# boyuanf/tensorflow_train_distributed

Hardware: AMD Instinct MI355X
Metric: images/sec (whole node) ResNet-50 bf16 MirroredStrategy at 1/2/4/8 MI355X (higher is better)
Workload: dtype bf16; 1 GPU; model=ResNet-50 v1.5, global_batch=1024, per_gpu_batch=1024, image_size=224, parallelism=dp1, optimizer=momentum-SGD 0.9, wd 5e-5, fp32 master, precision=bf16, hipgraph=True

## Files before the change

### tensorflow_train_distributed_amd/csrc/kernels/conv3_halo.hip

```cpp
#include "stream_epi.h"

namespace ttdk {
namespace {
namespace c3 {

constexpr int THR = 512;
constexpr int NW = THR / 64;

struct Pro {
  const bf16_t* x;
  const bf16_t* x2;
  const uint8_t* mask;
  const float* s;
  const float* b;
  bf16_t* side;
  uint8_t* side_mask;
};

__device__ __forceinline__ void load8f(const float* p, float (&d)[8]) {
  const f32x4_t a = *reinterpret_cast<const f32x4_t*>(p), c = *reinterpret_cast<const f32x4_t*>(p + 4);
#pragma unroll
  for (int j = 0; j < 4; ++j) {
    d[j] = a[j];
    d[4 + j] = c[j];
  }
}

template <int CP>
__device__ __forceinline__ int slot_chunk(int q) { return (q >> 3) % CP; }
template <int CP>
__device__ __forceinline__ int slot_pix(int q) { return (q & 7) + 8 * (q / (8 * CP)); }

template <int SCHED>
__device__ __forceinline__ int fresh(int tid) {
  if constexpr (SCHED != 0) {
    asm volatile("" : "+v"(tid));
    __builtin_assume(tid >= 0 && tid < THR);
  }
  return tid;
}

template <int SCHED>
__device__ __forceinline__ void frag_fence() {
  if constexpr (SCHED != 0) __builtin_amdgcn_sched_barrier(0);
}

template <int C, int BN, int TH, int W, int PRO, bool FLIP, int WM, int SCHED, int FEED>
__global__ __launch_bounds__(THR, 1) void conv3_kernel(Pro pa, const bf16_t* __restrict__ w, EpiParams E, int H,
                                                      int N, int tiles, int nslices) {
  constexpr int BM = TH * W;
  constexpr int HR = TH + 2, HC = W + 2;
  constexpr int CP = C / 8;
  constexpr int KT = 9 * C;
  constexpr int WN = NW / WM;
  constexpr int WR = BM / WM, WC = BN / WN;
  constexpr int TM = WR / 16, TN = WC / 16;
  constexpr int NPIX = HR * HC;
  constexpr int NCH = ((NPIX + 7) / 8) * 8 * CP;
  constexpr int NA = (NCH + THR - 1) / THR;
  constexpr int SB = BN * KT * 2;
  constexpr int REG = ((NPIX * 16 + 255) / 256) * 256;
  constexpr int SH = CP * REG;
  constexpr int PITCH = BN * 2 + 16;
  constexpr int SE = BM * PITCH + NW * 3 * BN * 4;
  constexpr int SAE = SH > SE ? SH : SE;
  static_assert(C % 64 == 0 && BN % 32 == 0 && WR % 16 == 0 && WC % 16 == 0, "tile shape");
  static_assert(THR % (8 * CP) == 0, "fixed channel chunk per thread");
  static_assert(SB + SAE <= 160 * 1024, "LDS budget");
  __shared__ __attribute__((aligned(16))) char smem[SB + SAE];
  char* const sB = smem;
  char* const sA = smem + SB;

  const int b = blockIdx.x;
  const int G = gridDim.x / nslices;
  const int xcd = b & 7, rq = b >> 3;
  const int slice = rq % nslices;
  const int per_xcd = G / 8;
  const int g = xcd * per_xcd + rq / nslices;
  const int n0 = slice * BN;
  const int tid = threadIdx.x, lane = tid & 63, wave = tid >> 6;
  const int wm = wave / WN, wn = wave % WN;
  const int tiles_per_img = H / TH;

  for (int q = tid; q < BN * (KT / 8); q += THR) {
    const int row = q / (KT / 8), kk = q % (KT / 8);
    const int tap = kk / CP, cc = kk % CP;
    const int n = n0 + row;
    const int src_tap = FLIP ? 8 - tap : tap;
    const uint4 v = n < N ? ldg16(w + (static_cast<long long>(n) * 9 + src_tap) * C + cc * 8) : make_uint4(0, 0, 0, 0);
    *reinterpret_cast<uint4*>(sB + (kk >> 3) * (BN * 128) + kmaj_off(row, kk & 7)) = v;
  }

  const int ac = slot_chunk<CP>(tid);
  const bool write_side = slice == 0 && pa.side != nullptr;

  const char* abase[TM];
#pragma unroll
  for (int a = 0; a < TM; ++a) {
    const int i = wm * WR + a * 16 + (lane & 15);
    abase[a] = sA + (lane >> 4) * REG + ((i / W) * HC + (i % W)) * 16;
  }

  uint4 ra[NA], rx[PRO == 2 ? NA : 1];
  uint32_t rm[(NA + 3) / 4];
  auto load_tile = [&](int t) {
    const int img = t / tiles_per_img, h0 = (t % tiles_per_img) * TH;
    const int ft = fresh<SCHED>(tid);
#pragma unroll
    for (int i = 0; i < (NA + 3) / 4; ++i) rm[i] = 0;
#pragma unroll
    for (int i = 0; i < NA; ++i) {
      const int pix = slot_pix<CP>(ft + THR * i);
      const int hr = pix / HC, hc = pix % HC;
      const int h = h0 - 1 + hr, x = hc - 1;
      const bool ok = pix < NPIX && h >= 0 && h < H && x >= 0 && x < W;
      const long long off = ((static_cast<long long>(img) * H + h) * W + x) * C + ac * 8;
      ra[i] = ok ? ldg16(pa.x + off) : make_uint4(0, 0, 0, 0);
      if constexpr (PRO == 2) {
        rx[i] = ok ? ldg16(pa.x2 + off) : make_uint4(0, 0, 0, 0);
        rm[i >> 2] |= static_cast<uint32_t>((ok && pa.mask) ? pa.mask[off >> 3] : 0xffu) << (8 * (i & 3));
      }
    }
  };
  auto stage_tile = [&](int t) {
    const int img = t / tiles_per_img, h0 = (t % tiles_per_img) * TH;
    float k0[8], k1[8], k2[8];
    if constexpr (PRO == 1) {
      load8f(pa.s + ac * 8, k0);
      load8f(pa.b + ac * 8, k1);
    } else if constexpr (PRO == 2) {
      load8f(pa.s + ac * 8, k0);
      load8f(pa.s + C + ac * 8, k1);
      load8f(pa.s + 2 * C + ac * 8, k2);
    }
    const int ft = fresh<SCHED>(tid);
#pragma unroll
    for (int i = 0; i < NA; ++i) {
      const int pix = slot_pix<CP>(ft + THR * i);
      if (ft + THR * i >= NCH) break;
      const int hr = pix / HC, hc = pix % HC;
      const int h = h0 - 1 + hr, x = hc - 1;
      const bool ok = h >= 0 && h < H && x >= 0 && x < W;
      const bool interior = ok && hr >= 1 && hr <= TH;
      const long long off = ((static_cast<long long>(img) * H + h) * W + x) * C + ac * 8;
      uint4 v = ra[i];
      if constexpr (PRO == 1) {
        float f[8];
        unpack8(ra[i], f);
#pragma unroll
        for (int j = 0; j < 8; ++j) f[j] = relu(f[j] * k0[j] + k1[j]);
        v = ok ? pack8(f) : make_uint4(0, 0, 0, 0);
        if (write_side && interior) {
          *reinterpret_cast<uint4*>(pa.side + off) = v;
          if (pa.side_mask) {
            const uint32_t wv[4] = {v.x, v.y, v.z, v.w};
            uint32_t mb = 0;
#pragma unroll
            for (int j = 0; j < 8; ++j) {
              const uint32_t hb = (wv[j >> 1] >> (16 * (j & 1))) & 0xffffu;
              mb |= ((hb & 0x7fffu) != 0 && !(hb & 0x8000u) ? 1u : 0u) << j;
            }
            pa.side_mask[off >> 3] = static_cast<uint8_t>(mb);
          }
        }
      } else if constexpr (PRO == 2) {
        float gq[8], yf[8];
        unpack8(ra[i], gq);
        const uint32_t mb = rm[i >> 2] >> (8 * (i & 3));
#pragma unroll
        for (int j = 0; j < 8; ++j) gq[j] = (mb >> j) & 1u ? gq[j] : 0.f;
        unpack8(rx[i], yf);
#pragma unroll
        for (int j = 0; j < 8; ++j) gq[j] = k0[j] * gq[j] + k1[j] * yf[j] + k2[j];
        v = ok ? pack8(gq) : make_uint4(0, 0, 0, 0);
        if (write_side && interior) *reinterpret_cast<uint4*>(pa.side + off) = v;
      }
      *reinterpret_cast<uint4*>(sA + ac * REG + pix * 16) = v;
    }
  };

  constexpr int ECPR = BN / 8;
  constexpr int RPP = THR / ECPR;
  constexpr int NR = (BM + RPP - 1) / RPP;
  constexpr int FA = NR >= 6 ? 3 : 2, FTAP = 6;
  static_assert(FEED == 0 || (FLIP && SCHED != 0), "feeding epilogue: data gradients under SCHED 1");
  const int M = tiles * BM;

  int t = g;
  if (t < tiles) load_tile(t);
  for (; t < tiles; t += G) {
    stage_tile(t);
    __syncthreads();
    if (t + G < tiles) load_tile(t + G);
    const int m0 = t * BM;
    sepi::FeedBatch<FA> fa;
    sepi::FeedBatch<NR - FA> fb;
    f32x4_t acc[TM][TN];
#pragma unroll
    for (int a = 0; a < TM; ++a)
#pragma unroll
      for (int c = 0; c < TN; ++c) acc[a][c] = f32x4_t{0.f, 0.f, 0.f, 0.f};
#pragma unroll
    for (int tap = 0; tap < 9; ++tap) {
      const int tq = (tap / 3) * HC + (tap % 3);
#pragma unroll
      for (int kc = 0; kc < C / 32; ++kc) {
        if constexpr (FEED != 0) {
          if (tap == FTAP && kc == 0) {
            const int ft = fresh<SCHED>(tid);
            sepi::feed_batch_load<BM, RPP, FA>(fa, E, 0, ft / ECPR, m0, M, n0 + (ft % ECPR) * 8);
          }
        }
        const int kglob = tap * C + kc * 32;
        const char* pB = sB + (kglob >> 6) * (BN * 128);
        const int kchunk = ((kglob & 63) >> 3) + (lane >> 4);
        bf16x8_t af[TM], bfr[TN];
#pragma unroll
        for (int c = 0; c < TN; ++c) {
          bfr[c] = lds_read_b128(pB + kmaj_off(wn * WC + c * 16 + (lane & 15), kchunk));
          frag_fence<SCHED>();
        }
#pragma unroll
        for (int a = 0; a < TM; ++a) {
          af[a] = lds_read_b128(abase[a] + kc * 4 * REG + tq * 16);
          frag_fence<SCHED>();
        }
#pragma unroll
        for (int a = 0; a < TM; ++a)
#pragma unroll
          for (int c = 0; c < TN; ++c) acc[a][c] = __builtin_amdgcn_mfma_f32_16x16x32_bf16(bfr[c], af[a], acc[a][c], 0, 0, 0);
        frag_fence<SCHED>();
      }
    }
    __syncthreads();
    const int fe = fresh<SCHED>(tid);
    const int c = fe % ECPR, r0 = fe / ECPR;
    const int n = n0 + c * 8;
    sepi::stage_acc<TM, TN, WR, WC, PITCH>(sA, acc, wm, wn, lane, epi_alpha(E));
    if constexpr (FEED != 0) sepi::feed_batch_load<BM, RPP, NR - FA>(fb, E, FA, r0, m0, M, n);
    __syncthreads();
    const bool nfull = n + 8 <= N;
    const bool vst = nfull && (E.ldo & 7) == 0;
    float bias8[8], s8[8], q8[8], r8[8];
#pragma unroll
    for (int j = 0; j < 8; ++j) {
      bias8[j] = (E.bias && n + j < N) ? E.bias[n + j] : 0.f;
      s8[j] = q8[j] = r8[j] = 0.f;
    }
    if constexpr (FEED != 0) {
      sepi::feed_batch_rows<BM, RPP, PITCH, FA>(fa, E, sA, 0, c, r0, m0, M, n, s8, q8);
      sepi::feed_batch_rows<BM, RPP, PITCH, NR - FA>(fb, E, sA, FA, c, r0, m0, M, n, s8, q8);
    } else if (E.beta || E.residual || E.by)
      epi_rows<BM, RPP, PITCH, true, 2>(E, sA, c, r0, n, m0, M, N, vst, vst, bias8, s8, q8, r8);
    else
      epi_rows<BM, RPP, PITCH, false>(E, sA, c, r0, n, m0, M, N, vst, vst, bias8, s8, q8, r8);
    if (E.stat)
      sepi::tile_stats<BN, NW, THR, ECPR>(E, reinterpret_cast<float*>(sA + BM * PITCH), s8, q8, r8, c, lane, wave, tid,
                                          n0, N, t);
    else
      __syncthreads();
  }
}

template <int C, int BN, int TH, int W, int PRO, bool FLIP, int WM, int SCHED, int FEED>
hipError_t launch(const Pro& pa, const bf16_t* w, const EpiParams& E, int Nimg, int H, int N, hipStream_t st) {
  const int nsl = N / BN;
  const int tiles = Nimg * (H / TH);
  int per_xcd = big::device_cus() / (8 * nsl);
  if (per_xcd < 1) per_xcd = 1;
  const int need = ceil_div(tiles, 8);
  if (per_xcd > need) per_xcd = need;
  hipLaunchKernelGGL((conv3_kernel<C, BN, TH, W, PRO, FLIP, WM, SCHED, FEED>), dim3(8 * nsl * per_xcd), dim3(THR), 0, st,
                     pa, w, E, H, N, tiles, nsl);
  return hipGetLastError();
}

inline int pick_th(int C, int N, int W, int pro) {
  if (C == 64 && N == 64 && W == 56) return pro == 2 ? 4 : 8;
  return 0;
}

template <int PRO, bool FLIP, int SCHED, int FEED>
hipError_t dispatch(const Pro& pa, const bf16_t* w, const EpiParams& E, int Nimg, int H, int W, int C, int N,
                    hipStream_t st) {
  if (C == 64 && N == 64 && W == 56) {
    if constexpr (PRO == 2) return launch<64, 64, 4, 56, PRO, FLIP, 2, SCHED, FEED>(pa, w, E, Nimg, H, N, st);
    else return launch<64, 64, 8, 56, PRO, FLIP, 4, SCHED, FEED>(pa, w, E, Nimg, H, N, st);
  }
  return hipErrorInvalidValue;
}

}

namespace c3s {

constexpr int THR = 512;
constexpr int NW = THR / 64;

__device__ __forceinline__ void dma16(const void* src, uint32_t lds_) {
  const uint32_t lds = __builtin_amdgcn_readfirstlane(lds_);
  unsigned keep;
  asm volatile("s_mov_b32 %0, m0\n\ts_mov_b32 m0, %2\n\ts_nop 0\n\tglobal_load_lds_dwordx4 %1, off\n\ts_mov_b32 m0, %0"
               : "=&s"(keep) : "v"(src), "s"(lds) : "memory");
}
__device__ __forceinline__ uint32_t lds_addr(const char* p) {
  typedef __attribute__((address_space(3))) const char lds_char_t;
  return (uint32_t)(size_t)(lds_char_t*)(p);
}

template <int N>
__device__ __forceinline__ void wait_vm() {
  asm volatile("s_waitcnt vmcnt(%0)" ::"n"(N) : "memory");
}
__device__ __forceinline__ void wait_vm_upto(int n) {
  switch (n) {
    case 1: wait_vm<1>(); break;
    case 2: wait_vm<2>(); break;
    case 3: wait_vm<3>(); break;
    default: wait_vm<0>(); break;
  }
}

template <int C, int BN, int TR, int H, int W, int PRO, bool FLIP, int SCHED, int FEED>
__global__ __launch_bounds__(THR, 1) void conv3s_kernel(c3::Pro pa, const bf16_t* __restrict__ w, EpiParams E,
                                                       int rows_total, int N, int tiles) {
  constexpr int WM = 2, WN = NW / WM;
  constexpr int BM = TR * W;
  constexpr int WR = BM / WM, WC = BN / WN;
  constexpr int TM = WR / 16, TN = WC / 16;
  constexpr int HS = TR + 4;
  constexpr int HC = W + 2;
  constexpr int NPIX = HS * HC;
  constexpr int CP = C / 8;
  constexpr int NCH = ((NPIX + 7) / 8) * 8 * CP;
  constexpr int NA = (NCH + THR - 1) / THR;
  constexpr int REG = ((NPIX * 16 + 255) / 256) * 256;
  constexpr int SH = CP * REG;
  constexpr int SBT = BN * C * 2;
  constexpr int PITCH = BN * 2 + 16;
  constexpr int SE = BM * PITCH + NW * 3 * BN * 4;
  constexpr int SAE = SH > SE ? SH : SE;
  constexpr int NDMA = SBT / 16 / THR;
  static_assert(PRO != 2 && C % 64 == 0 && BN % (16 * WN) == 0 && WR % 16 == 0 && TR <= H, "tile shape");
  static_assert(THR % (8 * CP) == 0 && SBT % (16 * THR) == 0, "staging / DMA mapping");
  static_assert(SAE + 2 * SBT <= 160 * 1024, "LDS budget");
  __shared__ __attribute__((aligned(16))) char smem[SAE + 2 * SBT];
  char* const sA = smem;
  char* const sBb = smem + SAE;

  const int b = blockIdx.x;
  const int G = gridDim.x;
  const int g = (b & 7) * (G / 8) + (b >> 3);
  const int tid = threadIdx.x, lane = tid & 63, wave = tid >> 6;
  const int wm = wave / WN, wn = wave % WN;
  const int ac = c3::slot_chunk<CP>(tid);
  const bool write_side = pa.side != nullptr;
  const int nimg = rows_total / H;

  const bf16_t* wsrc[NDMA];
#pragma unroll
  for (int i = 0; i < NDMA; ++i) {
    const int L = (i * NW + wave) * 64 + lane;
    const int sub = L / (BN * 8), p = L % (BN * 8), row = p >> 3, j = p & 7;
    const int sc = j ^ ((row >> 1) & 7);
    wsrc[i] = w + static_cast<long long>(row) * 9 * C + (sub * 8 + sc) * 8;
  }
  auto dma_tap = [&](int tap, int buf) {
    const int stap = FLIP ? 8 - tap : tap;
    char* dst = sBb + buf * SBT;
#pragma unroll
    for (int i = 0; i < NDMA; ++i) {
      if constexpr (SCHED != 0) {
        int off = stap * C;
        asm volatile("" : "+s"(off));
        dma16(wsrc[i] + off, lds_addr(dst + (i * NW + wave) * 1024));
      } else {
        const int L = (i * NW + wave) * 64 + lane;
        const int sub = L / (BN * 8), p = L % (BN * 8), row = p >> 3, j = p & 7;
        const int sc = j ^ ((row >> 1) & 7);
        dma16(w + (static_cast<long long>(row) * 9 + stap) * C + (sub * 8 + sc) * 8,
              lds_addr(dst + (i * NW + wave) * 1024));
      }
    }
  };
  struct Geo {
    int i0, h0, n0, n1;
  };
  auto geo = [&](int t) {
    Geo q;
    const int R0 = t * TR, R1 = min(R0 + TR, rows_total);
    q.i0 = R0 / H;
    q.h0 = R0 - q.i0 * H;
    q.n0 = min(R1, (q.i0 + 1) * H) - R0;
    q.n1 = R1 - R0 - q.n0;
    return q;
  };
  auto slot_src = [&](const Geo& q, int s, int& img, int& h, bool& interior) {
    if (s < q.n0 + 2) {
      img = q.i0;
      h = q.h0 - 1 + s;
      interior = s >= 1 && s <= q.n0;
      return true;
    }
    const int u = s - (q.n0 + 2);
    img = q.i0 + 1;
    h = u - 1;
    interior = u >= 1 && u <= q.n1;
    return q.n1 > 0 && u < q.n1 + 2;
  };

  uint4 ra[NA];
  auto load_slot = [&](const Geo& q, int ft, int i) {
    const int qq = ft + THR * i;
    const int pix = c3::slot_pix<CP>(qq);
    const int s = pix / HC, x = pix % HC - 1;
    int img, h;
    bool interior;
    const bool ok = qq < NCH && slot_src(q, s, img, h, interior) && h >= 0 && h < H && x >= 0 && x < W;
    const long long off = ((static_cast<long long>(img) * H + h) * W + x) * C + ac * 8;
    ra[i] = ldg16(ok ? pa.x + off : reinterpret_cast<const bf16_t*>(big::g_zero));
  };
  auto load_tile = [&](int t) {
    const Geo q = geo(t);
    const int ft = c3::fresh<SCHED>(tid);
#pragma unroll
    for (int i = 0; i < NA; ++i) load_slot(q, ft, i);
  };
  auto stage_tile = [&](int t) {
    const Geo q = geo(t);
    float k0[8], k1[8];
    if constexpr (PRO == 1) {
      c3::load8f(pa.s + ac * 8, k0);
      c3::load8f(pa.b + ac * 8, k1);
    }
    const int ft = c3::fresh<SCHED>(tid);
#pragma unroll
    for (int i = 0; i < NA; ++i) {
      const int qq = ft + THR * i;
      if (qq >= NCH) break;
      const int pix = c3::slot_pix<CP>(qq);
      const int s = pix / HC, x = pix % HC - 1;
      int img, h;
      bool interior;
      const bool ok = slot_src(q, s, img, h, interior) && h >= 0 && h < H && x >= 0 && x < W;
      uint4 v = ok ? ra[i] : make_uint4(0, 0, 0, 0);
      if constexpr (PRO == 1) {
        const long long off = ((static_cast<long long>(img) * H + h) * W + x) * C + ac * 8;
        float f[8];
        unpack8(ra[i], f);
#pragma unroll
        for (int j = 0; j < 8; ++j) f[j] = relu(f[j] * k0[j] + k1[j]);
        v = ok ? pack8(f) : make_uint4(0, 0, 0, 0);
        if (write_side && ok && interior) {
          *reinterpret_cast<uint4*>(pa.side + off) = v;
          if (pa.side_mask) {
            const uint32_t wv[4] = {v.x, v.y, v.z, v.w};
            uint32_t mb = 0;
#pragma unroll
            for (int j = 0; j < 8; ++j) {
              const uint32_t hb = (wv[j >> 1] >> (16 * (j & 1))) & 0xffffu;
              mb |= ((hb & 0x7fffu) != 0 && !(hb & 0x8000u) ? 1u : 0u) << j;
            }
            pa.side_mask[off >> 3] = static_cast<uint8_t>(mb);
          }
        }
      }
      *reinterpret_cast<uint4*>(sA + ac * REG + pix * 16) = v;
    }
  };

  constexpr int ECPR = BN / 8;
  constexpr int RPP = THR / ECPR;
  constexpr int NR = (BM + RPP - 1) / RPP;
  constexpr int FA = 3, FTAP = 9 - FA;
  static_assert(NR > FA, "two batches");
  static_assert(FEED == 0 || (FLIP && SCHED != 0), "feeding epilogue: data gradients under SCHED 1");
  const int M = rows_total * W;

  int bcur = 0;
  int t = g;
  if (t < tiles) {
    dma_tap(0, 0);
    load_tile(t);
    if constexpr (SCHED != 0) wait_vm<0>();
  }
  for (; t < tiles; t += G) {
    const Geo q = geo(t);
    int abase[TM];
#pragma unroll
    for (int a = 0; a < TM; ++a) {
      const int i = wm * WR + a * 16 + (lane & 15);
      const int j = i / W, col = i % W;
      abase[a] = (lane >> 4) * REG + ((j + (j >= q.n0 ? 2 : 0)) * HC + col) * 16;
    }
    stage_tile(t);
    if constexpr (SCHED == 0) wait_vm<0>();
    __syncthreads();
    const bool more = t + G < tiles;
    sepi::FeedBatch<1> fa[FA];
    sepi::FeedBatch<NR - FA> fb;
    f32x4_t acc[TM][TN];
#pragma unroll
    for (int a = 0; a < TM; ++a)
#pragma unroll
      for (int c = 0; c < TN; ++c) acc[a][c] = f32x4_t{0.f, 0.f, 0.f, 0.f};
    constexpr int HPT = 2;
    static_assert(HPT * 8 >= NA, "the halo loads are all retired by the wait of the last tap");
    static_assert(HPT * FTAP >= NA, "no tap issues both halo and feeding loads (wait_vm_upto takes 0 .. 3)");
    const int m0 = t * BM;
    const Geo qn = geo(SCHED != 0 && more ? t + G : t);
#pragma unroll(SCHED != 0 ? 9 : 1)
    for (int tap = 0; tap < 9; ++tap) {
      const int bnext = bcur ^ 1;
      if (tap < 8) dma_tap(tap + 1, bnext);
      else if (more) dma_tap(0, bnext);
      const int h0 = tap * HPT < NA ? tap * HPT : NA, h1 = h0 + HPT < NA ? h0 + HPT : NA;
      if constexpr (SCHED != 0) {
        if (more) {
          const int ft = c3::fresh<SCHED>(tid);
#pragma unroll
          for (int i = h0; i < h1; ++i) load_slot(qn, ft, i);
        }
      }
      const int nfeed = (FEED != 0 && tap >= FTAP) ? 2 : 0;
      if constexpr (FEED != 0) {
        if (tap >= FTAP) {
          const int ft = c3::fresh<SCHED>(tid);
          sepi::feed_batch_load<BM, RPP, 1>(fa[tap - FTAP], E, tap - FTAP, ft / ECPR, m0, M, (ft % ECPR) * 8);
        }
      }
      const char* sBc = sBb + bcur * SBT;
      const int tq = ((tap / 3) * HC + (tap % 3)) * 16;
#pragma unroll
      for (int kc = 0; kc < C / 32; ++kc) {
        const int kglob = kc * 32;
        const char* pB = sBc + (kglob >> 6) * (BN * 128);
        const int kchunk = ((kglob & 63) >> 3) + (lane >> 4);
        bf16x8_t af[TM], bfr[TN];
#pragma unroll
        for (int c = 0; c < TN; ++c) {
          bfr[c] = lds_read_b128(pB + kmaj_off(wn * WC + c * 16 + (lane & 15), kchunk));
          c3::frag_fence<SCHED>();
        }
#pragma unroll
        for (int a = 0; a < TM; ++a) {
          af[a] = lds_read_b128(sA + abase[a] + kc * 4 * REG + tq);
          c3::frag_fence<SCHED>();
        }
#pragma unroll
        for (int a = 0; a < TM; ++a)
#pragma unroll
          for (int c = 0; c < TN; ++c) acc[a][c] = __builtin_amdgcn_mfma_f32_16x16x32_bf16(bfr[c], af[a], acc[a][c], 0, 0, 0);
        c3::frag_fence<SCHED>();
      }
      if constexpr (SCHED != 0) wait_vm_upto((more ? h1 - h0 : 0) + nfeed);
      else wait_vm<0>();
      __syncthreads();
      bcur = bnext;
    }
    const int fe = c3::fresh<SCHED>(tid);
    const int c = fe % ECPR, r0 = fe / ECPR;
    const int n = c * 8;
    sepi::stage_acc<TM, TN, WR, WC, PITCH>(sA, acc, wm, wn, lane, epi_alpha(E));
    if constexpr (FEED != 0) sepi::feed_batch_load<BM, RPP, NR - FA>(fb, E, FA, r0, m0, M, n);
    if constexpr (SCHED == 0)
      if (more) load_tile(t + G);
    __syncthreads();
    const bool vst = (E.ldo & 7) == 0;
    float bias8[8], s8[8], q8[8], r8[8];
#pragma unroll
    for (int j = 0; j < 8; ++j) {
      bias8[j] = E.bias ? E.bias[n + j] : 0.f;
      s8[j] = q8[j] = r8[j] = 0.f;
    }
    if constexpr (FEED != 0) {
#pragma unroll
      for (int k = 0; k < FA; ++k) sepi::feed_batch_rows<BM, RPP, PITCH, 1>(fa[k], E, sA, k, c, r0, m0, M, n, s8, q8);
      sepi::feed_batch_rows<BM, RPP, PITCH, NR - FA>(fb, E, sA, FA, c, r0, m0, M, n, s8, q8);
    } else if (E.beta || E.residual || E.by)
      epi_rows<BM, RPP, PITCH, true, 2>(E, sA, c, r0, n, m0, M, N, vst, vst, bias8, s8, q8, r8);
    else
      epi_rows<BM, RPP, PITCH, false>(E, sA, c, r0, n, m0, M, N, vst, vst, bias8, s8, q8, r8);
    if (E.stat)
      sepi::tile_stats<BN, NW, THR, ECPR>(E, reinterpret_cast<float*>(sA + BM * PITCH), s8, q8, r8, c, lane, wave, tid,
                                          0, N, t);
    else
      __syncthreads();
    (void)nimg;
  }
}

template <int PRO, bool FLIP, int SCHED, int FEED>
hipError_t launch(const c3::Pro& pa, const bf16_t* w, const EpiParams& E, int Nimg, int N, hipStream_t st) {
  const int rows = Nimg * 28;
  const int tiles = ceil_div(rows, 8);
  int G = big::device_cus() / 8 * 8;
  if (G < 8) G = 8;
  const int need = ceil_div(tiles, 8) * 8;
  if (G > need) G = need;
  hipLaunchKernelGGL((conv3s_kernel<128, 128, 8, 28, 28, PRO, FLIP, SCHED, FEED>), dim3(G), dim3(THR), 0, st, pa, w, E,
                     rows, N, tiles);
  return hipGetLastError();
}

inline bool fits(int H, int W, int C, int N, int pro) { return C == 128 && N == 128 && H == 28 && W == 28 && pro != 2; }

}
}
}

using namespace ttdk;

namespace {
int& conv3_s3_flag() {
  static int on = getenv_int("TTD_CONV3_S3", 1);
  return on;
}
int& conv3_sched_flag() {
  static int on = getenv_int("TTD_CONV3_SCHED", 1);
  return on;
}
int& conv3_feed_flag() {
  static int on = getenv_int("TTD_CONV3_FEED", 1);
  return on;
}
}

TTDK_EXPORT int ttdk_set_conv3_feed(int on) {
  const int old = conv3_feed_flag();
  conv3_feed_flag() = on ? 1 : 0;
  return old;
}

TTDK_EXPORT int ttdk_set_conv3_sched(int on) {
  const int old = conv3_sched_flag();
  conv3_sched_flag() = on ? 1 : 0;
  return old;
}

TTDK_EXPORT int ttdk_set_conv3_s3(int on) {
  const int old = conv3_s3_flag();
  conv3_s3_flag() = on;
  return old;
}

TTDK_EXPORT int ttdk_conv3_rows(int H, int W, int C, int N, int pro) {
  if (conv3_s3_flag() && c3s::fits(H, W, C, N, pro)) return 8 * W;
  const int th = c3::pick_th(C, N, W, pro);
  return (th && H % th == 0) ? th * W : 0;
}

TTDK_EXPORT int ttdk_conv3_halo(const bf16_t* x, const bf16_t* x2, const uint8_t* mask_in, const float* s,
                                const float* b, bf16_t* side, uint8_t* side_mask, int pro, int flip, const bf16_t* w,
                                int Nimg, int H, int W, int C, int N, const TtdkEpilogue* epi, hipStream_t st) {
  const int sched = conv3_sched_flag();
  if (ttdk_conv3_rows(H, W, C, N, pro) == 8 * W && c3s::fits(H, W, C, N, pro)) {
    if ((reinterpret_cast<uintptr_t>(x) & 15) || (reinterpret_cast<uintptr_t>(w) & 15)) return hipErrorInvalidValue;
    const EpiParams e = to_epi(epi);
    if (e.mode != 0 || e.remap || e.bH || e.ldo != N || e.residual || e.by2) return hipErrorInvalidValue;
    if (pro == 1 && (!s || !b)) return hipErrorInvalidValue;
    if (side_mask && pro != 1) return hipErrorInvalidValue;
    const c3::Pro pa{x, nullptr, nullptr, s, b, side, side_mask};
    if (pro == 0 && flip && sched && conv3_feed_flag() && sepi::feed_case(e))
      return c3s::launch<0, true, 1, 1>(pa, w, e, Nimg, N, st);
#define C3S_CASE(P_, F_)              \
  if (pro == P_ && (flip != 0) == F_) \
    return sched ? c3s::launch<P_, F_, 1, 0>(pa, w, e, Nimg, N, st) : c3s::launch<P_, F_, 0, 0>(pa, w, e, Nimg, N, st);
    C3S_CASE(0, false)
    C3S_CASE(0, true)
    C3S_CASE(1, false)
#undef C3S_CASE
    return hipErrorInvalidValue;
  }
  const int th = c3::pick_th(C, N, W, pro);
  if (!th || H % th || (reinterpret_cast<uintptr_t>(x) & 15) || pro < 0 || pro > 2) return hipErrorInvalidValue;
  const EpiParams e = to_epi(epi);
  if (e.mode != 0 || e.remap || e.bH || e.ldo != N || e.residual || e.by2) return hipErrorInvalidValue;
  if (pro == 1 && (!s || !b)) return hipErrorInvalidValue;
  if (pro == 2 && (!s || !x2)) return hipErrorInvalidValue;
  if (side_mask && pro != 1) return hipErrorInvalidValue;
  const c3::Pro pa{x, x2, mask_in, s, b, side, side_mask};
  if (flip && sched && conv3_feed_flag() && sepi::feed_case(e)) {
    if (pro == 0) return c3::dispatch<0, true, 1, 1>(pa, w, e, Nimg, H, W, C, N, st);
    if (pro == 2) return c3::dispatch<2, true, 1, 1>(pa, w, e, Nimg, H, W, C, N, st);
  }
#define C3_CASE(P_, F_)                                                        \
  if (pro == P_ && (flip != 0) == F_)                                          \
    return sched ? c3::dispatch<P_, F_, 1, 0>(pa, w, e, Nimg, H, W, C, N, st)  \
                 : c3::dispatch<P_, F_, 0, 0>(pa, w, e, Nimg, H, W, C, N, st);
  C3_CASE(0, false)
  C3_CASE(1, false)
  C3_CASE(0, true)
  C3_CASE(2, true)
#undef C3_CASE
  return hipErrorInvalidValue;
}
```

### tensorflow_train_distributed_amd/ops/gemm.py

```python
from __future__ import annotations

import ctypes

import torch

from . import _lib, _plan

ACT_NONE, ACT_RELU, ACT_GELU, ACT_TANH, ACT_DGELU = 0, 1, 2, 3, 4

import os as _os
_LOG = [] if _os.environ.get("TTD_GEMM_LOG") else None


def gemm_log(reset=False):
    out = list(_LOG or [])
    if reset and _LOG is not None:
        _LOG.clear()
    return out


def _log(kind, M, N, K, splits=1):
    if _LOG is not None:
        _LOG.append((kind, int(M), int(N), int(K), int(splits)))
    _lib.label((kind, int(M), int(N), int(K)))
# ... 151 lines not shown
    _lib.call("ttdk_gemm_bf16_batched", a.data_ptr(), a.stride(1), a.stride(0), 0 if trans_a else 1, b.data_ptr(),
              b.stride(1), b.stride(0), 1 if trans_b else 0, out.data_ptr(), N, M * N,
              1 if out_dtype == torch.float32 else 0, M, N, K, Bt, _lib.stream())
    return out


def wgrad_bias_ok(M, N, K, splits) -> bool:
    if M % 8 or N % 8 or K % 64:
        return False
    if int(_lib.query("ttdk_gemm_wgrad_bias_ws", int(M), int(N), int(K), int(splits))) < 0:
        return False
    kt = K // 64
    return -(-kt // _plan.clamp_splits(kt, int(splits))) >= 16


def gemm_wgrad_bias(dy, x, out, bias_out, splits=1, beta=0, alpha=1.0):
    _check2d(dy, torch.bfloat16, "dy")
    _check2d(x, torch.bfloat16, "x")
    K, M = dy.shape
    K2, N = x.shape
    if K != K2:
        raise ValueError("gemm_wgrad_bias: token dims differ (%d vs %d)" % (K, K2))
    if tuple(out.shape) != (M, N) or out.dtype != torch.float32 or not out.is_contiguous():
        raise ValueError("gemm_wgrad_bias: out must be a contiguous fp32 [%d, %d]" % (M, N))
    if bias_out.numel() != M or bias_out.dtype != torch.float32 or not bias_out.is_contiguous():
        raise ValueError("gemm_wgrad_bias: bias_out must be a contiguous fp32 [%d]" % M)
    nws = int(_lib.query("ttdk_gemm_wgrad_bias_ws", M, N, K, int(splits)))
    if nws < 0:
        raise ValueError("gemm_wgrad_bias: shape %dx%dx%d not on the 256-wide kernel" % (M, N, K))
    ws = torch.empty(nws, dtype=torch.float32, device=dy.device)
    _log("wgrad_bias", M, N, K, splits)
    _lib.call("ttdk_gemm_wgrad_bias", dy.data_ptr(), dy.stride(0), x.data_ptr(), x.stride(0), M, N, K, int(splits),
              ws.data_ptr(), out.data_ptr(), int(beta), float(alpha), bias_out.data_ptr(), _lib.stream())
    return out, bias_out


def gemm4t(dy, x, out=None, bias_out=None, *, splits=1, beta=0, alpha=1.0):
    _check2d(dy, torch.bfloat16, "dy")
    _check2d(x, torch.bfloat16, "x")
    K, M = dy.shape
    K2, N = x.shape
    if K != K2:
        raise ValueError("gemm4t: token dims differ (%d vs %d)" % (K, K2))
    if out is None:
        out = torch.empty((M, N), dtype=torch.float32, device=dy.device)
    if tuple(out.shape) != (M, N) or out.dtype != torch.float32 or not out.is_contiguous():
        raise ValueError("gemm4t: out must be a contiguous fp32 [%d, %d]" % (M, N))
    if bias_out is not None and (bias_out.numel() != M or bias_out.dtype != torch.float32
                                 or not bias_out.is_contiguous()):
        raise ValueError("gemm4t: bias_out must be a contiguous fp32 [%d]" % M)
    nws = int(_lib.query("ttdk_gemm4t_ws", M, N, K, int(splits)))
    if nws < 0:
        raise ValueError("gemm4t does not take M=%d N=%d K=%d (K a multiple of 64 >= 128, M / N multiples "
                         "of 8, operands < 2 GiB, TTD_G4T on)" % (M, N, K))
    ws = torch.empty(max(nws, 1), dtype=torch.float32, device=dy.device)
    _log("gemm4t", M, N, K, splits)
    _lib.call("ttdk_gemm4t_wgrad", dy.data_ptr(), dy.stride(0), x.data_ptr(), x.stride(0), M, N, K, int(splits),
              ws.data_ptr(), out.data_ptr(), int(beta), float(alpha), _lib.ptr(bias_out), _lib.stream())
    return out


_C3 = _os.environ.get("TTD_CONV3", "1") != "0"


_lib.register({"ttdk_set_conv3_s3": [_lib.I]})


def set_conv3_s3(on: bool) -> bool:
    return bool(_lib.query("ttdk_set_conv3_s3", 1 if on else 0))


_lib.register({"ttdk_set_conv3_sched": [_lib.I]})


def set_conv3_sched(new: bool) -> bool:
    return bool(_lib.query("ttdk_set_conv3_sched", 1 if new else 0))


_lib.register({"ttdk_set_conv3_feed": [_lib.I]})


def set_conv3_feed(new: bool) -> bool:
    return bool(_lib.query("ttdk_set_conv3_feed", 1 if new else 0))


def conv3_rows(H, W, C, N, pro=0):
    return int(_lib.query("ttdk_conv3_rows", int(H), int(W), int(C), int(N), int(pro))) if _C3 else 0


def conv3_halo(x, w, *, prologue=None, flip=False, out=None, stat=False, bn_stat=None):
    _check(x, torch.bfloat16, "x")
    _check(w, torch.bfloat16, "w")
    Nimg, H, W, C = x.shape
    Co = w.shape[0]
    if tuple(w.shape) != (Co, 3, 3, C):
        raise ValueError("conv3_halo: filter must be [%d, 3, 3, %d], got %s" % (Co, C, tuple(w.shape)))
    pro_code = 0 if prologue is None else {"bn_fwd": 1, "bn_bwd": 2}.get(prologue[0], -1)
    bm = conv3_rows(H, W, C, Co, max(pro_code, 0))
    if not bm:
        raise ValueError("conv3_halo: shape %s -> %d not compiled in" % (tuple(x.shape), Co))
    if out is None:
        out = torch.empty((Nimg, H, W, Co), dtype=torch.bfloat16, device=x.device)
    T = -(-Nimg * H * W // bm)
    partial = None
    by = bmask = None
    if stat or bn_stat is not None:
        partial = torch.empty((T, 2, Co), dtype=torch.float32, device=x.device)
    if bn_stat is not None:
        by, bmask = bn_stat
        _check(by, torch.bfloat16, "bn_stat y")
    e = _epi(out, ldo=Co, stat=partial, by=by, bmask=bmask)
    P = _lib.ptr
    pro, x2, mask_in, s, b, side, side_mask = 0, None, None, None, None, None, None
    if prologue is not None:
        if prologue[0] == "bn_fwd":
            _, s, b, side, side_mask = prologue
            pro = 1
        elif prologue[0] == "bn_bwd":
            _, x2, mask_in, s, side = prologue
            pro = 2
        else:
            raise ValueError("unknown prologue %r" % (prologue[0],))
    _log("c3_%s" % ("dgrad" if flip else "fwd"), Nimg * H * W, Co, 9 * C)
    _lib.call("ttdk_conv3_halo", x.data_ptr(), P(x2), P(mask_in), P(s), P(b), P(side), P(side_mask), pro, int(flip),
              w.data_ptr(), Nimg, H, W, C, Co, ctypes.byref(e), _lib.stream())
    if partial is not None:
        return out, partial, T
    return out


def gemm_f32(a, b, *, trans_a=False, trans_b=False, out=None, bias=None, beta=0):
    _check2d(a, torch.float32, "a")
    _check2d(b, torch.float32, "b")
    M, K = (a.shape[1], a.shape[0]) if trans_a else a.shape
    Kb, N = (b.shape[1], b.shape[0]) if trans_b else b.shape
    if K != Kb:
        raise ValueError("gemm inner dims differ: %d vs %d" % (K, Kb))
    if out is None:
        if beta:
            raise ValueError("beta=1 needs an out tensor")
        out = torch.empty((M, N), dtype=torch.float32, device=a.device)
    elif out.dtype != torch.float32 or tuple(out.shape) != (M, N) or out.stride(-1) != 1:
        raise ValueError("gemm_f32 out must be fp32 [%d, %d] row-major" % (M, N))
    if bias is not None:
        _check(bias, torch.float32, "bias")
    _log("gemm_f32_%s%s" % ("t" if trans_a else "n", "t" if trans_b else "n"), M, N, K, 1)
    _lib.call("ttdk_gemm_f32", a.data_ptr(), a.stride(0), int(trans_a), b.data_ptr(), b.stride(0), int(trans_b),
              out.data_ptr(), out.stride(0), _lib.ptr(bias), int(bool(beta)), M, N, K, _lib.stream())
    return out


BIG_WGRAD_WGS = int(_os.environ.get("TTD_WGRAD_WGS", "128"))


def gemm_wgrad_splits(M, N, K, target_blocks=1024, min_ktiles=8, big_wgs=None):
    bbn = big_bn(M, N, K)
    if bbn:
        tiles = -(-M // 256) * -(-N // bbn)
        return max(1, min((K // 64) // 32, -(-(big_wgs or BIG_WGRAD_WGS) // tiles)))
    bm, bn = _plan.pick_tile(M, N)
    tiles = -(-M // bm) * -(-N // bn)
    ktiles = -(-K // 64)
    return max(1, min(ktiles // min_ktiles, -(-target_blocks // tiles)))


def conv_geom(x_shape, w_shape, stride, padding, dilation=(1, 1)):
# ... 641 lines not shown
```

Measured before the change: 16030 images/sec.

## Interleave BN-ReLU prologue of next conv3 tile with current tile's MFMA loop

Adds a split-staging variant (STG) of the forward 3x3 conv kernels with a BN+ReLU prologue. The next tile's halo is loaded, normalized, activated and written to the side buffer and mask slot by slot between MFMA k-steps. Only plain register-to-LDS stores remain before the barrier, which takes prologue ALU work off the critical path between tiles. It also adds a simplified plain-epilogue store path, and gates the variant with an env flag that defaults to on for the 56x56 kernel (the 28x28 one needs level 2). The cost is higher register pressure and more complex scheduling inside the MFMA loop.

```diff
diff --git a/tensorflow_train_distributed_amd/csrc/kernels/conv3_halo.hip b/tensorflow_train_distributed_amd/csrc/kernels/conv3_halo.hip
--- a/tensorflow_train_distributed_amd/csrc/kernels/conv3_halo.hip
+++ b/tensorflow_train_distributed_amd/csrc/kernels/conv3_halo.hip
@@ -45,7 +45,63 @@
   if constexpr (SCHED != 0) __builtin_amdgcn_sched_barrier(0);
 }
 
-template <int C, int BN, int TH, int W, int PRO, bool FLIP, int WM, int SCHED, int FEED>
+__device__ __forceinline__ uint4 bn_relu8(const uint4& x, const float (&k0)[8], const float (&k1)[8]) {
+  float f[8];
+  unpack8(x, f);
+#pragma unroll
+  for (int j = 0; j < 8; ++j) f[j] = relu(f[j] * k0[j] + k1[j]);
+  return pack8(f);
+}
+__device__ __forceinline__ uint32_t relu_bits8(const uint4& v) {
+  const uint32_t wv[4] = {v.x, v.y, v.z, v.w};
+  uint32_t mb = 0;
+#pragma unroll
+  for (int j = 0; j < 8; ++j) {
+    const uint32_t hb = (wv[j >> 1] >> (16 * (j & 1))) & 0xffffu;
+    mb |= ((hb & 0x7fffu) != 0 && !(hb & 0x8000u) ? 1u : 0u) << j;
+  }
+  return mb;
+}
+__device__ __forceinline__ uint2 gather_bits8(uint32_t mb) {
+  mb |= static_cast<uint32_t>(__shfl_xor(static_cast<int>(mb), 8, 64)) << 8;
+  mb |= static_cast<uint32_t>(__shfl_xor(static_cast<int>(mb), 16, 64)) << 16;
+  return make_uint2(mb, static_cast<uint32_t>(__shfl_xor(static_cast<int>(mb), 32, 64)));
+}
+
+__device__ __forceinline__ void landed(uint4& v) {
+  asm volatile("" : "+v"(v.x), "+v"(v.y), "+v"(v.z), "+v"(v.w));
+}
+__device__ __forceinline__ void landed(float (&k)[8]) {
+#pragma unroll
+  for (int j = 0; j < 8; ++j) asm volatile("" : "+v"(k[j]));
+}
+
+template <int BM, int RPP, int PITCH>
+__device__ __forceinline__ void plain_rows(const EpiParams& E, const char* smem, int c, int r0, int n, int m0, int M,
+                                           float (&s8)[8], float (&q8)[8]) {
+  bf16_t* op = static_cast<bf16_t*>(E.out) + static_cast<long long>(m0 + r0) * E.ldo + n;
+  const long long step = static_cast<long long>(RPP) * E.ldo;
+  const int rmax = min(BM, M - m0);
+#pragma unroll 4
+  for (int r = r0; r < rmax; r += RPP, op += step) {
+    const uint4 v = *reinterpret_cast<const uint4*>(smem + r * PITCH + c * 16);
+    *reinterpret_cast<uint4*>(op) = v;
+    if (E.stat) {
+      float sv[8];
+      unpack8(v, sv);
+#pragma unroll
+      for (int j = 0; j < 8; ++j) {
+        s8[j] += sv[j];
+        q8[j] += sv[j] * sv[j];
+      }
+    }
+  }
+}
+inline bool plain_epi(const EpiParams& e) {
+  return !e.bias && !e.residual && !e.aux && e.act == kActNone && !e.remap && !e.beta && !e.by && (e.ldo & 7) == 0;
+}
+
+template <int C, int BN, int TH, int W, int PRO, bool FLIP, int WM, int SCHED, int FEED, int STG>
 __global__ __launch_bounds__(THR, 1) void conv3_kernel(Pro pa, const bf16_t* __restrict__ w, EpiParams E, int H,
                                                       int N, int tiles, int nslices) {
   constexpr int BM = TH * W;
@@ -103,7 +159,7 @@
 
   uint4 ra[NA], rx[PRO == 2 ? NA : 1];
   uint32_t rm[(NA + 3) / 4];
-  auto load_tile = [&](int t) {
+  auto load_tile = [&](int t, bool live = true) {
     const int img = t / tiles_per_img, h0 = (t % tiles_per_img) * TH;
     const int ft = fresh<SCHED>(tid);
 #pragma unroll
@@ -113,9 +169,10 @@
       const int pix = slot_pix<CP>(ft + THR * i);
       const int hr = pix / HC, hc = pix % HC;
       const int h = h0 - 1 + hr, x = hc - 1;
-      const bool ok = pix < NPIX && h >= 0 && h < H && x >= 0 && x < W;
+      const bool ok = live && pix < NPIX && h >= 0 && h < H && x >= 0 && x < W;
       const long long off = ((static_cast<long long>(img) * H + h) * W + x) * C + ac * 8;
-      ra[i] = ok ? ldg16(pa.x + off) : make_uint4(0, 0, 0, 0);
+      if constexpr (STG != 0) ra[i] = ldg16(ok ? pa.x + off : reinterpret_cast<const bf16_t*>(big::g_zero));
+      else ra[i] = ok ? ldg16(pa.x + off) : make_uint4(0, 0, 0, 0);
       if constexpr (PRO == 2) {
         rx[i] = ok ? ldg16(pa.x2 + off) : make_uint4(0, 0, 0, 0);
         rm[i >> 2] |= static_cast<uint32_t>((ok && pa.mask) ? pa.mask[off >> 3] : 0xffu) << (8 * (i & 3));
@@ -178,6 +235,31 @@
       *reinterpret_cast<uint4*>(sA + ac * REG + pix * 16) = v;
     }
   };
+  static_assert(STG == 0 || (PRO == 1 && !FLIP && SCHED != 0 && FEED == 0), "split staging: PRO 1 forward under SCHED 1");
+  static_assert(STG == 0 || NA <= 9 * (C / 32), "one slot per k-step");
+  float k0[STG != 0 ? 8 : 1], k1[STG != 0 ? 8 : 1];
+  auto pro_slot = [&](bool live, int img, int h0, int i) {
+    if constexpr (STG != 0) {
+      const int qq = fresh<SCHED>(tid) + THR * i;
+      const int pix = slot_pix<CP>(qq);
+      const int hr = pix / HC, hc = pix % HC;
+      const int h = h0 - 1 + hr, x = hc - 1;
+      const bool ok = live && qq < NCH && pix < NPIX && h >= 0 && h < H && x >= 0 && x < W;
+      const uint4 v = ok ? bn_relu8(ra[i], k0, k1) : make_uint4(0, 0, 0, 0);
+      ra[i] = v;
+      const uint2 bits = gather_bits8(relu_bits8(v));
+      if (write_side && ok && hr >= 1 && hr <= TH) {
+        const long long base = (static_cast<long long>(img) * H + h0 - 1) * (W * C);
+        const int lo = (hr * W + x) * C + ac * 8;
+        *reinterpret_cast<uint4*>(pa.side + base + lo) = v;
+        if (pa.side_mask && (ac & 7) == 0) *reinterpret_cast<uint2*>(pa.side_mask + ((base + lo) >> 3)) = bits;
+      }
+    }
+  };
+  auto put_slot = [&](int i) {
+    const int qq = fresh<SCHED>(tid) + THR * i;
+    if (qq < NCH) *reinterpret_cast<uint4*>(sA + ac * REG + slot_pix<CP>(qq) * 16) = ra[i];
+  };
 
   constexpr int ECPR = BN / 8;
   constexpr int RPP = THR / ECPR;
@@ -187,11 +269,30 @@
   const int M = tiles * BM;
 
   int t = g;
-  if (t < tiles) load_tile(t);
+  if (t < tiles) {
+    load_tile(t);
+    if constexpr (STG != 0) {
+      load8f(pa.s + ac * 8, k0);
+      load8f(pa.b + ac * 8, k1);
+      landed(k0);
+      landed(k1);
+#pragma unroll
+      for (int i = 0; i < NA; ++i) pro_slot(true, t / tiles_per_img, (t % tiles_per_img) * TH, i);
+    }
+  }
   for (; t < tiles; t += G) {
-    stage_tile(t);
+    if constexpr (STG != 0) {
+#pragma unroll
+      for (int i = 0; i < NA; ++i) put_slot(i);
+    } else {
+      stage_tile(t);
+    }
     __syncthreads();
-    if (t + G < tiles) load_tile(t + G);
+    const bool more = t + G < tiles;
+    if constexpr (STG != 0) load_tile(more ? t + G : t, more);
+    else if (more) load_tile(t + G);
+    const int img_n = STG != 0 && more ? (t + G) / tiles_per_img : 0;
+    const int h0_n = STG != 0 && more ? ((t + G) % tiles_per_img) * TH : 0;
     const int m0 = t * BM;
     sepi::FeedBatch<FA> fa;
     sepi::FeedBatch<NR - FA> fb;
@@ -230,6 +331,11 @@
 #pragma unroll
           for (int c = 0; c < TN; ++c) acc[a][c] = __builtin_amdgcn_mfma_f32_16x16x32_bf16(bfr[c], af[a], acc[a][c], 0, 0, 0);
         frag_fence<SCHED>();
+        if constexpr (STG != 0) {
+          constexpr int KS = C / 32;
+          const int sl = tap * KS + kc - (9 * KS - NA);
+          if (sl >= 0) pro_slot(more, img_n, h0_n, sl);
+        }
       }
     }
     __syncthreads();
@@ -250,6 +356,8 @@
     if constexpr (FEED != 0) {
       sepi::feed_batch_rows<BM, RPP, PITCH, FA>(fa, E, sA, 0, c, r0, m0, M, n, s8, q8);
       sepi::feed_batch_rows<BM, RPP, PITCH, NR - FA>(fb, E, sA, FA, c, r0, m0, M, n, s8, q8);
+    } else if constexpr (STG != 0) {
+      if (n < N) c3::plain_rows<BM, RPP, PITCH>(E, sA, c, r0, n, m0, M, s8, q8);
     } else if (E.beta || E.residual || E.by)
       epi_rows<BM, RPP, PITCH, true, 2>(E, sA, c, r0, n, m0, M, N, vst, vst, bias8, s8, q8, r8);
     else
@@ -262,7 +370,7 @@
   }
 }
 
-template <int C, int BN, int TH, int W, int PRO, bool FLIP, int WM, int SCHED, int FEED>
+template <int C, int BN, int TH, int W, int PRO, bool FLIP, int WM, int SCHED, int FEED, int STG>
 hipError_t launch(const Pro& pa, const bf16_t* w, const EpiParams& E, int Nimg, int H, int N, hipStream_t st) {
   const int nsl = N / BN;
   const int tiles = Nimg * (H / TH);
@@ -270,7 +378,7 @@
   if (per_xcd < 1) per_xcd = 1;
   const int need = ceil_div(tiles, 8);
   if (per_xcd > need) per_xcd = need;
-  hipLaunchKernelGGL((conv3_kernel<C, BN, TH, W, PRO, FLIP, WM, SCHED, FEED>), dim3(8 * nsl * per_xcd), dim3(THR), 0, st,
+  hipLaunchKernelGGL((conv3_kernel<C, BN, TH, W, PRO, FLIP, WM, SCHED, FEED, STG>), dim3(8 * nsl * per_xcd), dim3(THR), 0, st,
                      pa, w, E, H, N, tiles, nsl);
   return hipGetLastError();
 }
@@ -280,12 +388,12 @@
   return 0;
 }
 
-template <int PRO, bool FLIP, int SCHED, int FEED>
+template <int PRO, bool FLIP, int SCHED, int FEED, int STG = 0>
 hipError_t dispatch(const Pro& pa, const bf16_t* w, const EpiParams& E, int Nimg, int H, int W, int C, int N,
                     hipStream_t st) {
   if (C == 64 && N == 64 && W == 56) {
-    if constexpr (PRO == 2) return launch<64, 64, 4, 56, PRO, FLIP, 2, SCHED, FEED>(pa, w, E, Nimg, H, N, st);
-    else return launch<64, 64, 8, 56, PRO, FLIP, 4, SCHED, FEED>(pa, w, E, Nimg, H, N, st);
+    if constexpr (PRO == 2) return launch<64, 64, 4, 56, PRO, FLIP, 2, SCHED, FEED, STG>(pa, w, E, Nimg, H, N, st);
+    else return launch<64, 64, 8, 56, PRO, FLIP, 4, SCHED, FEED, STG>(pa, w, E, Nimg, H, N, st);
   }
   return hipErrorInvalidValue;
 }
@@ -321,7 +429,7 @@
   }
 }
 
-template <int C, int BN, int TR, int H, int W, int PRO, bool FLIP, int SCHED, int FEED>
+template <int C, int BN, int TR, int H, int W, int PRO, bool FLIP, int SCHED, int FEED, int STG>
 __global__ __launch_bounds__(THR, 1) void conv3s_kernel(c3::Pro pa, const bf16_t* __restrict__ w, EpiParams E,
                                                        int rows_total, int N, int tiles) {
   constexpr int WM = 2, WN = NW / WM;
@@ -410,13 +518,13 @@
   };
 
   uint4 ra[NA];
-  auto load_slot = [&](const Geo& q, int ft, int i) {
+  auto load_slot = [&](const Geo& q, int ft, int i, bool live = true) {
     const int qq = ft + THR * i;
     const int pix = c3::slot_pix<CP>(qq);
     const int s = pix / HC, x = pix % HC - 1;
     int img, h;
     bool interior;
-    const bool ok = qq < NCH && slot_src(q, s, img, h, interior) && h >= 0 && h < H && x >= 0 && x < W;
+    const bool ok = live && qq < NCH && slot_src(q, s, img, h, interior) && h >= 0 && h < H && x >= 0 && x < W;
     const long long off = ((static_cast<long long>(img) * H + h) * W + x) * C + ac * 8;
     ra[i] = ldg16(ok ? pa.x + off : reinterpret_cast<const bf16_t*>(big::g_zero));
   };
@@ -468,6 +576,31 @@
       *reinterpret_cast<uint4*>(sA + ac * REG + pix * 16) = v;
     }
   };
+  static_assert(STG == 0 || (PRO == 1 && !FLIP && SCHED != 0 && FEED == 0), "split staging: PRO 1 forward under SCHED 1");
+  float k0[STG != 0 ? 8 : 1], k1[STG != 0 ? 8 : 1];
+  auto pro_slot = [&](bool live, const Geo& q, int i) {
+    if constexpr (STG != 0) {
+      const int qq = c3::fresh<SCHED>(tid) + THR * i;
+      const int pix = c3::slot_pix<CP>(qq);
+      const int s = pix / HC, x = pix % HC - 1;
+      int img, h;
+      bool interior;
+      const bool ok = live && qq < NCH && slot_src(q, s, img, h, interior) && h >= 0 && h < H && x >= 0 && x < W;
+      const uint4 v = ok ? c3::bn_relu8(ra[i], k0, k1) : make_uint4(0, 0, 0, 0);
+      ra[i] = v;
+      const uint2 bits = c3::gather_bits8(c3::relu_bits8(v));
+      if (write_side && ok && interior) {
+        const long long base = static_cast<long long>(q.i0) * (H * W * C);
+        const int lo = (((img - q.i0) * H + h) * W + x) * C + ac * 8;
+        *reinterpret_cast<uint4*>(pa.side + base + lo) = v;
+        if (pa.side_mask && (ac & 7) == 0) *reinterpret_cast<uint2*>(pa.side_mask + ((base + lo) >> 3)) = bits;
+      }
+    }
+  };
+  auto put_slot = [&](int i) {
+    const int qq = c3::fresh<SCHED>(tid) + THR * i;
+    if (qq < NCH) *reinterpret_cast<uint4*>(sA + ac * REG + c3::slot_pix<CP>(qq) * 16) = ra[i];
+  };
 
   constexpr int ECPR = BN / 8;
   constexpr int RPP = THR / ECPR;
@@ -480,9 +613,20 @@
   int bcur = 0;
   int t = g;
   if (t < tiles) {
+    if constexpr (STG != 0) {
+      c3::load8f(pa.s + ac * 8, k0);
+      c3::load8f(pa.b + ac * 8, k1);
+      c3::landed(k0);
+      c3::landed(k1);
+    }
     dma_tap(0, 0);
     load_tile(t);
     if constexpr (SCHED != 0) wait_vm<0>();
+    if constexpr (STG != 0) {
+      const Geo q0 = geo(t);
+#pragma unroll
+      for (int i = 0; i < NA; ++i) pro_slot(true, q0, i);
+    }
   }
   for (; t < tiles; t += G) {
     const Geo q = geo(t);
@@ -493,7 +637,12 @@
       const int j = i / W, col = i % W;
       abase[a] = (lane >> 4) * REG + ((j + (j >= q.n0 ? 2 : 0)) * HC + col) * 16;
     }
-    stage_tile(t);
+    if constexpr (STG != 0) {
+#pragma unroll
+      for (int i = 0; i < NA; ++i) put_slot(i);
+    } else {
+      stage_tile(t);
+    }
     if constexpr (SCHED == 0) wait_vm<0>();
     __syncthreads();
     const bool more = t + G < tiles;
@@ -507,19 +656,31 @@
     constexpr int HPT = 2;
     static_assert(HPT * 8 >= NA, "the halo loads are all retired by the wait of the last tap");
     static_assert(HPT * FTAP >= NA, "no tap issues both halo and feeding loads (wait_vm_upto takes 0 .. 3)");
+    static_assert(STG == 0 || HPT * 7 >= NA, "STG 1: slots loaded in tap k are applied in tap k + 2 <= 8");
     const int m0 = t * BM;
     const Geo qn = geo(SCHED != 0 && more ? t + G : t);
 #pragma unroll(SCHED != 0 ? 9 : 1)
     for (int tap = 0; tap < 9; ++tap) {
       const int bnext = bcur ^ 1;
+      const int p0 = (STG != 0 && tap >= 2 && (tap - 2) * HPT < NA) ? (tap - 2) * HPT : NA;
+      const int p1 = p0 + HPT < NA ? p0 + HPT : NA;
+      if constexpr (STG != 0) {
+#pragma unroll
+        for (int i = p0; i < p1; ++i) c3::landed(ra[i]);
+      }
       if (tap < 8) dma_tap(tap + 1, bnext);
       else if (more) dma_tap(0, bnext);
+      if constexpr (STG != 0) {
+#pragma unroll
+        for (int i = p0; i < p1; ++i) pro_slot(more, qn, i);
+      }
+      const bool lds = more || STG != 0;
       const int h0 = tap * HPT < NA ? tap * HPT : NA, h1 = h0 + HPT < NA ? h0 + HPT : NA;
       if constexpr (SCHED != 0) {
-        if (more) {
+        if (lds) {
           const int ft = c3::fresh<SCHED>(tid);
 #pragma unroll
-          for (int i = h0; i < h1; ++i) load_slot(qn, ft, i);
+          for (int i = h0; i < h1; ++i) load_slot(qn, ft, i, more);
         }
       }
       const int nfeed = (FEED != 0 && tap >= FTAP) ? 2 : 0;
@@ -553,7 +714,7 @@
           for (int c = 0; c < TN; ++c) acc[a][c] = __builtin_amdgcn_mfma_f32_16x16x32_bf16(bfr[c], af[a], acc[a][c], 0, 0, 0);
         c3::frag_fence<SCHED>();
       }
-      if constexpr (SCHED != 0) wait_vm_upto((more ? h1 - h0 : 0) + nfeed);
+      if constexpr (SCHED != 0) wait_vm_upto((lds ? h1 - h0 : 0) + nfeed);
       else wait_vm<0>();
       __syncthreads();
       bcur = bnext;
@@ -577,6 +738,8 @@
 #pragma unroll
       for (int k = 0; k < FA; ++k) sepi::feed_batch_rows<BM, RPP, PITCH, 1>(fa[k], E, sA, k, c, r0, m0, M, n, s8, q8);
       sepi::feed_batch_rows<BM, RPP, PITCH, NR - FA>(fb, E, sA, FA, c, r0, m0, M, n, s8, q8);
+    } else if constexpr (STG != 0) {
+      if (n < N) c3::plain_rows<BM, RPP, PITCH>(E, sA, c, r0, n, m0, M, s8, q8);
     } else if (E.beta || E.residual || E.by)
       epi_rows<BM, RPP, PITCH, true, 2>(E, sA, c, r0, n, m0, M, N, vst, vst, bias8, s8, q8, r8);
     else
@@ -590,7 +753,7 @@
   }
 }
 
-template <int PRO, bool FLIP, int SCHED, int FEED>
+template <int PRO, bool FLIP, int SCHED, int FEED, int STG = 0>
 hipError_t launch(const c3::Pro& pa, const bf16_t* w, const EpiParams& E, int Nimg, int N, hipStream_t st) {
   const int rows = Nimg * 28;
   const int tiles = ceil_div(rows, 8);
@@ -598,7 +761,7 @@
   if (G < 8) G = 8;
   const int need = ceil_div(tiles, 8) * 8;
   if (G > need) G = need;
-  hipLaunchKernelGGL((conv3s_kernel<128, 128, 8, 28, 28, PRO, FLIP, SCHED, FEED>), dim3(G), dim3(THR), 0, st, pa, w, E,
+  hipLaunchKernelGGL((conv3s_kernel<128, 128, 8, 28, 28, PRO, FLIP, SCHED, FEED, STG>), dim3(G), dim3(THR), 0, st, pa, w, E,
                      rows, N, tiles);
   return hipGetLastError();
 }
@@ -624,6 +787,17 @@
   static int on = getenv_int("TTD_CONV3_FEED", 1);
   return on;
 }
+int clamp_stage(int v) { return v < 0 ? 0 : v > 2 ? 2 : v; }
+int& conv3_stage_flag() {
+  static int on = clamp_stage(getenv_int("TTD_CONV3_STAGE", 1));
+  return on;
+}
+}
+
+TTDK_EXPORT int ttdk_set_conv3_stage(int on) {
+  const int old = conv3_stage_flag();
+  conv3_stage_flag() = clamp_stage(on);
+  return old;
 }
 
 TTDK_EXPORT int ttdk_set_conv3_feed(int on) {
@@ -654,6 +828,7 @@
                                 const float* b, bf16_t* side, uint8_t* side_mask, int pro, int flip, const bf16_t* w,
                                 int Nimg, int H, int W, int C, int N, const TtdkEpilogue* epi, hipStream_t st) {
   const int sched = conv3_sched_flag();
+  const bool stg_ok = sched && pro == 1 && !flip && (reinterpret_cast<uintptr_t>(side_mask) & 7) == 0;
   if (ttdk_conv3_rows(H, W, C, N, pro) == 8 * W && c3s::fits(H, W, C, N, pro)) {
     if ((reinterpret_cast<uintptr_t>(x) & 15) || (reinterpret_cast<uintptr_t>(w) & 15)) return hipErrorInvalidValue;
     const EpiParams e = to_epi(epi);
@@ -663,6 +838,7 @@
     const c3::Pro pa{x, nullptr, nullptr, s, b, side, side_mask};
     if (pro == 0 && flip && sched && conv3_feed_flag() && sepi::feed_case(e))
       return c3s::launch<0, true, 1, 1>(pa, w, e, Nimg, N, st);
+    if (stg_ok && conv3_stage_flag() >= 2 && c3::plain_epi(e)) return c3s::launch<1, false, 1, 0, 1>(pa, w, e, Nimg, N, st);
 #define C3S_CASE(P_, F_)              \
   if (pro == P_ && (flip != 0) == F_) \
     return sched ? c3s::launch<P_, F_, 1, 0>(pa, w, e, Nimg, N, st) : c3s::launch<P_, F_, 0, 0>(pa, w, e, Nimg, N, st);
@@ -684,6 +860,7 @@
     if (pro == 0) return c3::dispatch<0, true, 1, 1>(pa, w, e, Nimg, H, W, C, N, st);
     if (pro == 2) return c3::dispatch<2, true, 1, 1>(pa, w, e, Nimg, H, W, C, N, st);
   }
+  if (stg_ok && conv3_stage_flag() >= 1 && c3::plain_epi(e)) return c3::dispatch<1, false, 1, 0, 1>(pa, w, e, Nimg, H, W, C, N, st);
 #define C3_CASE(P_, F_)                                                        \
   if (pro == P_ && (flip != 0) == F_)                                          \
     return sched ? c3::dispatch<P_, F_, 1, 0>(pa, w, e, Nimg, H, W, C, N, st)  \
diff --git a/tensorflow_train_distributed_amd/ops/gemm.py b/tensorflow_train_distributed_amd/ops/gemm.py
--- a/tensorflow_train_distributed_amd/ops/gemm.py
+++ b/tensorflow_train_distributed_amd/ops/gemm.py
@@ -257,6 +257,13 @@
 
 def set_conv3_feed(new: bool) -> bool:
     return bool(_lib.query("ttdk_set_conv3_feed", 1 if new else 0))
+
+
+_lib.register({"ttdk_set_conv3_stage": [_lib.I]})
+
+
+def set_conv3_stage(new: int) -> int:
+    return int(_lib.query("ttdk_set_conv3_stage", int(new)))
 
 
 def conv3_rows(H, W, C, N, pro=0):
```

Result: no change. 16120 images/sec (median of 6 runs) (+0.6%).
